# prs-eth/ResDepth

Measured on AMD Instinct MI355X. Metric: DSM tiles/sec fwd+bwd (256x256, 3-ch, depth-5 U-Net), higher is better.
Workload: dtype f32

## Files before the change

### resdepth_amd/csrc/rd_igemm.hip

```cpp
#include <stdlib.h>
#include <string.h>

#include <type_traits>

#include "rd_common.h"
#include "rd_mfma_dev.h"
#include "rd_nt.h"

namespace rd {

template <int BM, int BN, int WM, int WN, int AMODE, int EPI>
__global__ __launch_bounds__(256) void igemm_nt_kernel(NtParams p) {
    constexpr int BK = 32, LS = BK + 4;
    constexpr int TM = BM / WM / 32, TN = BN / WN / 32;
    constexpr int AI = BM / 32, BI = BN / 32;
    __shared__ __attribute__((aligned(16))) float smem[(BM + BN) * LS];
    float* As = smem;
    float* Bs = smem + BM * LS;

    const int lb = xcd_remap(blockIdx.x, gridDim.x);
    const int tile_n = lb % p.tiles_n, tile_m = lb / p.tiles_n;
    const int m0 = tile_m * BM, n0 = tile_n * BN;
    const int t = threadIdx.x, lane = t & 63, wave = t >> 6;
    const int wm = wave / WN, wn = wave % WN;
// ... 1090 lines not shown
        __syncthreads();
        for (long kb = k_begin; kb < k_end; kb += BK) {
            const bool more = kb + BK < k_end;
            if (more) load_tile(kb + BK);
#pragma unroll
            for (int ks = 0; ks < BK / 2; ++ks) {
                float af[TM], bf[TN];
#pragma unroll
                for (int i = 0; i < TM; ++i) af[i] = a_base[ks * 2 * BM + i * 32];
#pragma unroll
                for (int j = 0; j < TN; ++j) bf[j] = b_base[ks * 2 * BN + j * 32];
#pragma unroll
                for (int i = 0; i < TM; ++i)
#pragma unroll
                    for (int j = 0; j < TN; ++j)
                        acc[i][j] = __builtin_amdgcn_mfma_f32_32x32x2f32(af[i], bf[j], acc[i][j], 0, 0, 0);
            }
            __syncthreads();
            if (more) {
                store_tile();
                __syncthreads();
            }
        }
    }

    float* out = p.slab + (long)split * p.M * p.N;
#pragma unroll
    for (int i = 0; i < TM; ++i)
#pragma unroll
        for (int j = 0; j < TN; ++j) {
            const int n = n0 + wn * TN * 32 + j * 32 + lrow;
            if (n >= p.N) continue;
#pragma unroll
            for (int r = 0; r < 16; ++r) {
                const int m = m0 + wm * TM * 32 + i * 32 + (r & 3) + 8 * (r >> 2) + 4 * half;
                if (m < p.M) out[(long)m * p.N + n] = acc[i][j][r];
            }
        }
}

template <int NP, int BM, int BN, int WM, int WN, int AMODE, int BMODE>
__device__ __forceinline__ void wgrad_tn_split_body(const TnParams& p, float* smem, const Quant qz) {
    typedef typename frag_of<NP>::type FR;
    constexpr int NT = NP == 3 ? 2 : 3;
    constexpr int TM = BM / WM / 32, TN = BN / WN / 32;
    constexpr int STAGE = (BM + BN) * 32;

    const int nb_mn = p.tiles_mn;
    const int gb = xcd_remap(blockIdx.x, gridDim.x);
    const int split = gb / nb_mn;
    const int lb = gb - split * nb_mn;
    const int tile_n = lb % p.tiles_n, tile_m = lb / p.tiles_n;
    const int m0 = tile_m * BM, n0 = tile_n * BN;
    const int t = threadIdx.x, lane = t & 63, wave = t >> 6;
    const int wm = wave / WN, wn = wave % WN;
    const int H = p.H, W = p.W;

    const bool isA = t < BM, active = t < BM + BN;
    const int idx = isA ? t : t - BM;
    const int kq = idx & 3, quad = idx >> 2;
    const int col0 = (isA ? m0 : n0) + quad * 4;
    const bool col_ok = active && col0 < (isA ? p.M : p.N);
    int a_col = col0, a_qa = 0, a_qb = 0;
    if (AMODE == WA_UP2 && isA) {
        const int ab = col0 / p.Cout;
        a_col = col0 - ab * p.Cout;
        a_qa = ab >> 1;
        a_qb = ab & 1;
    }
    int b_col = col0, b_dy = 0, b_dx = 0;
    if (BMODE == WB_CONV3 && !isA) {
        const int tap = col0 / p.Cin;
        b_col = col0 - tap * p.Cin;
        b_dy = tap / 3 - 1;
        b_dx = tap - (tap / 3) * 3 - 1;
    }
    const int b_shift = b_dy * W + b_dx;
    const int lds_row0 = (isA ? 0 : BM) + quad * 4;

    f32x16 acc[TM][TN], lo[TM][TN];
#pragma unroll
    for (int i = 0; i < TM; ++i)
#pragma unroll
        for (int j = 0; j < TN; ++j)
#pragma unroll
            for (int r = 0; r < 16; ++r) acc[i][j][r] = lo[i][j][r] = 0.f;

    const long k_begin = (long)split * p.kchunk;
    long k_end = k_begin + p.kchunk;
    if (k_end > p.Kp) k_end = p.Kp;
    const __amdgpu_buffer_rsrc_t rsA = make_rsrc(p.A, p.a_bytes), rsB = make_rsrc(p.B, p.b_bytes);

    const bool w4 = (W & 3) == 0;
    auto load_task = [&](long kbase, float4 (&x)[4]) {
        const int rem = (int)(k_end - kbase);
        int img0 = 0, y0 = 0, x0 = 0;
        if ((AMODE == WA_UP2 && isA) || (BMODE == WB_CONV3 && !isA)) pix_split((int)kbase + kq * 4, p.pd, img0, y0, x0);
        unsigned up_off0 = 0;
        const unsigned up_step = (unsigned)(2 * p.lda * 4);
        if (AMODE == WA_UP2 && isA && w4)
            up_off0 = (unsigned)(((((long)img0 * (2 * H) + 2 * y0 + a_qa) * (2 * W) + 2 * x0 + a_qb) * p.lda + a_col) * 4);
#pragma unroll
        for (int j = 0; j < 4; ++j) {
            const int row = kq * 4 + j;
            const bool ok = col_ok && row < rem;
            if (isA) {
                if (AMODE == WA_UP2) {
                    unsigned off = up_off0 + j * up_step;
                    if (!w4) {
                        int jj, ii, img;
                        pix_split((int)kbase + row, p.pd, img, ii, jj);
                        off = (unsigned)(((((long)img * (2 * H) + 2 * ii + a_qa) * (2 * W) + 2 * jj + a_qb) * p.lda + a_col) * 4);
                    }
                    x[j] = buf_load4(rsA, ok ? off : kOOB, 0);
                } else {
                    x[j] = buf_load4(rsA, ok ? (unsigned)((row * p.lda + a_col) * 4) : kOOB, (unsigned)(kbase * p.lda * 4));
                }
            } else {
                if (BMODE == WB_CONV3) {
                    const int m = (int)kbase + row;
                    int y = y0, xx = x0 + j, img_ = img0;
                    if (!w4) pix_split(m, p.pd, img_, y, xx);
                    const bool in = ok && ((unsigned)(y + b_dy) < (unsigned)H) && ((unsigned)(xx + b_dx) < (unsigned)W);
                    x[j] = buf_load4(rsB, in ? (unsigned)((((long)m + b_shift) * p.ldb + b_col) * 4) : kOOB, 0);
                } else {
                    x[j] = buf_load4(rsB, ok ? (unsigned)((row * p.ldb + b_col) * 4) : kOOB, (unsigned)(kbase * p.ldb * 4));
                }
            }
        }
    };
    const float qs = __uint_as_float((unsigned)__builtin_amdgcn_readfirstlane((int)__float_as_uint(isA ? qz.sa : qz.sb)));
    auto store_task = [&](float* stage, const float4 (&x)[4]) {
        if (!active) return;
#pragma unroll
        for (int c = 0; c < 4; ++c) {
            uint2 ph, pm, pl;
            split_pack4v<NP, false>(c == 0 ? x[0].x : c == 1 ? x[0].y : c == 2 ? x[0].z : x[0].w, c == 0 ? x[1].x : c == 1 ? x[1].y : c == 2 ? x[1].z : x[1].w,
                                c == 0 ? x[2].x : c == 1 ? x[2].y : c == 2 ? x[2].z : x[2].w, c == 0 ? x[3].x : c == 1 ? x[3].y : c == 2 ? x[3].z : x[3].w,
                                qs, ph, pm, pl);
            const int row = lds_row0 + c;
            const int sw = (row >> 1) & 7;
            float* base = stage + row * 32 + (kq & 1) * 2;
            const int hi = kq >> 1;
            *reinterpret_cast<uint2*>(base + ((0 + hi) ^ sw) * 4) = ph;
            *reinterpret_cast<uint2*>(base + ((2 + hi) ^ sw) * 4) = pm;
            if (kterm3<NP>()) *reinterpret_cast<uint2*>(base + ((4 + hi) ^ sw) * 4) = pl;
        }
    };

    const int lrow = lane & 31, half = lane >> 5;
    int a_rd[TM][3], b_rd[TN][3];
#pragma unroll
    for (int i = 0; i < TM; ++i) {
        const int row = (wm * TM + i) * 32 + lrow;
#pragma unroll
        for (int q = 0; q < 3; ++q) a_rd[i][q] = row * 32 + ((2 * q + half) ^ ((row >> 1) & 7)) * 4;
    }
#pragma unroll
    for (int j = 0; j < TN; ++j) {
        const int row = BM + (wn * TN + j) * 32 + lrow;
#pragma unroll
        for (int q = 0; q < 3; ++q) b_rd[j][q] = row * 32 + ((2 * q + half) ^ ((row >> 1) & 7)) * 4;
    }
    auto mma_tile = [&](const float* stage) {
        FR af[TM][3], bf[TN][3];
#pragma unroll
        for (int i = 0; i < TM; ++i)
#pragma unroll
            for (int q = 0; q < NT; ++q) af[i][q] = *reinterpret_cast<const FR*>(stage + a_rd[i][q]);
#pragma unroll
        for (int j = 0; j < TN; ++j)
#pragma unroll
            for (int q = 0; q < NT; ++q) bf[j][q] = *reinterpret_cast<const FR*>(stage + b_rd[j][q]);
#pragma unroll
        for (int t6 = lo0<NP>(); t6 < 5; ++t6)
#pragma unroll
            for (int i = 0; i < TM; ++i)
#pragma unroll
                for (int j = 0; j < TN; ++j) lo[i][j] = mfma16<NP>(af[i][PA6[t6]], bf[j][PB6[t6]], lo[i][j]);
#pragma unroll
        for (int i = 0; i < TM; ++i)
#pragma unroll
            for (int j = 0; j < TN; ++j) acc[i][j] = mfma16<NP>(af[i][0], bf[j][0], acc[i][j]);
    };

    if (k_begin < k_end) {
        float* st0 = smem;
        float* st1 = smem + STAGE;
        float4 x0[4], x1[4];
        load_task(k_begin, x0);
        load_task(k_begin + SK, x1);
        store_task(st0, x0);
        __syncthreads();
        for (long kb = k_begin; kb < k_end; kb += 2 * SK) {
            load_task(kb + 2 * SK, x0);
            mma_tile(st0);
            store_task(st1, x1);
            __syncthreads();
            load_task(kb + 3 * SK, x1);
            mma_tile(st1);
            store_task(st0, x0);
            __syncthreads();
        }
    }

    float* out = p.slab + (long)split * p.M * p.N;
#pragma unroll
    for (int i = 0; i < TM; ++i)
#pragma unroll
        for (int j = 0; j < TN; ++j) {
            const int n = n0 + wn * TN * 32 + j * 32 + lrow;
            if (n >= p.N) continue;
#pragma unroll
            for (int r = 0; r < 16; ++r) {
                const int m = m0 + wm * TM * 32 + i * 32 + (r & 3) + 8 * (r >> 2) + 4 * half;
                if (m < p.M) out[(long)m * p.N + n] = merge_q<NP>(acc[i][j][r], lo[i][j][r], qz.dexp);
            }
        }
}

template <int BM, int BN, int WM, int WN, int AMODE, int BMODE>
__global__ __launch_bounds__(256) void wgrad_tn_split_kernel(TnParams p) {
    __shared__ __attribute__((aligned(16))) float smem[2 * (BM + BN) * 32];
    const Quant qz = quant_select(p.a_amax, p.b_amax);
    if (qz.use3) wgrad_tn_split_body<3, BM, BN, WM, WN, AMODE, BMODE>(p, smem, qz);
    else wgrad_tn_split_body<6, BM, BN, WM, WN, AMODE, BMODE>(p, smem, qz);
}

struct TnPlan {
    int bm, bn, tiles_m, tiles_n, splits, kchunk;
};

static TnPlan plan_tn(int M, int N, long Kp) {
    TnPlan pl;
    pl.bm = M > 64 ? 128 : 64;
    pl.bn = N > 64 ? 128 : 64;
    const int tforce = tune(TUNE_TN_TILE);
    if (tforce > 0) {
        pl.bm = tforce / 1000;
        pl.bn = tforce % 1000;
    }
    pl.tiles_m = cdiv(M, pl.bm);
    pl.tiles_n = cdiv(N, pl.bn);
    const int tiles = pl.tiles_m * pl.tiles_n;
    long ktiles = (Kp + 31) / 32;
    const int target = tune(TUNE_TN_BLOCKS);
    long want = target / tiles;
    if (want < 1) want = 1;
    long maxs = ktiles / 8 > 0 ? ktiles / 8 : 1;
    long s = want < maxs ? want : maxs;
    if (s < 1) s = 1;
    if (s > 512) s = 512;
    long per = (ktiles + s - 1) / s;
    pl.kchunk = (int)(per * 32);
    pl.splits = (int)((ktiles + per - 1) / per);
    return pl;
}

template <int AMODE, int BMODE>
static int launch_tn(TnParams p, const TnPlan& pl, hipStream_t s, const char* cls) {
    char pcls[64];
    const int tn_force = tune(TUNE_TN_SPLIT);
    const int split = tn_force >= 0 ? tn_force : (mfma_split() && pl.bm == 128 && pl.bn == 128);
    snprintf(pcls, sizeof(pcls), "%s|wgrad_tn%s<%d,%d,%d,%d>", cls, split ? "_split" : "", pl.bm, pl.bn, AMODE, BMODE);
    ProfScope ps(s, pcls, 2.0 * p.M * p.N * (double)p.Kp,
                 4.0 * ((double)p.Kp * p.lda * (AMODE == WA_UP2 ? 4 : 1) + (double)p.Kp * p.ldb + (double)p.M * p.N), true);
    const double a_bytes = 4.0 * (double)p.Kp * p.lda * (AMODE == WA_UP2 ? 4 : 1), b_bytes = 4.0 * (double)p.Kp * p.ldb;
    if (a_bytes >= 4294967040.0 || b_bytes >= 4294967040.0) {
        set_error("%s: operand larger than the 4 GiB buffer-descriptor range", cls);
        return RD_ERR_ARG;
    }
    p.a_bytes = (unsigned)a_bytes;
    p.b_bytes = (unsigned)b_bytes;
    p.kchunk = pl.kchunk;
    p.tiles_n = pl.tiles_n;
    p.tiles_mn = pl.tiles_m * pl.tiles_n;
    if (!split || mfma_products() != 3 || !p.a_amax || !p.b_amax) p.a_amax = p.b_amax = nullptr;
    const int grid = p.tiles_mn * pl.splits;
    if (split) {
        if (pl.bm == 128 && pl.bn == 128)
            RD_LAUNCH((wgrad_tn_split_kernel<128, 128, 2, 2, AMODE, BMODE>), dim3(grid), dim3(256), 0, s, p);
        else if (pl.bm == 128)
            RD_LAUNCH((wgrad_tn_split_kernel<128, 64, 2, 2, AMODE, BMODE>), dim3(grid), dim3(256), 0, s, p);
        else if (pl.bn == 128)
            RD_LAUNCH((wgrad_tn_split_kernel<64, 128, 2, 2, AMODE, BMODE>), dim3(grid), dim3(256), 0, s, p);
        else
            RD_LAUNCH((wgrad_tn_split_kernel<64, 64, 2, 2, AMODE, BMODE>), dim3(grid), dim3(256), 0, s, p);
        RD_LAUNCH_CHECK(cls);
        return RD_OK;
    }
    if (pl.bm == 128 && pl.bn == 128)
        RD_LAUNCH((wgrad_tn_kernel<128, 128, 2, 2, AMODE, BMODE>), dim3(grid), dim3(256), 0, s, p);
    else if (pl.bm == 128)
        RD_LAUNCH((wgrad_tn_kernel<128, 64, 2, 2, AMODE, BMODE>), dim3(grid), dim3(256), 0, s, p);
    else if (pl.bn == 128)
        RD_LAUNCH((wgrad_tn_kernel<64, 128, 2, 2, AMODE, BMODE>), dim3(grid), dim3(256), 0, s, p);
    else
        RD_LAUNCH((wgrad_tn_kernel<64, 64, 2, 2, AMODE, BMODE>), dim3(grid), dim3(256), 0, s, p);
    RD_LAUNCH_CHECK(cls);
    return RD_OK;
}

template <int SPT>
__global__ __launch_bounds__(256) void slab_reduce_kernel(const float* __restrict__ slab, float* __restrict__ dw, int M,
                                                          int N, int splits, int mode, int Cin, int Cout) {
    const long total = (long)M * N, quads = total >> 2;
    const long nthreads = (long)gridDim.x * blockDim.x;
    for (long gid = (long)blockIdx.x * blockDim.x + threadIdx.x; gid < quads * SPT; gid += nthreads) {
        const long q = gid / SPT;
        const int part = (int)(gid - q * SPT);
        const float4* src = reinterpret_cast<const float4*>(slab) + q;
        double a0 = 0.0, a1 = 0.0, a2 = 0.0, a3 = 0.0;
        int s = part;
        for (; s + 3 * SPT < splits; s += 4 * SPT) {
            const float4 v0 = src[(long)s * quads], v1 = src[(long)(s + SPT) * quads];
            const float4 v2 = src[(long)(s + 2 * SPT) * quads], v3 = src[(long)(s + 3 * SPT) * quads];
            a0 += ((double)v0.x + (double)v1.x) + ((double)v2.x + (double)v3.x);
            a1 += ((double)v0.y + (double)v1.y) + ((double)v2.y + (double)v3.y);
            a2 += ((double)v0.z + (double)v1.z) + ((double)v2.z + (double)v3.z);
            a3 += ((double)v0.w + (double)v1.w) + ((double)v2.w + (double)v3.w);
        }
        for (; s < splits; s += SPT) {
            const float4 v = src[(long)s * quads];
            a0 += v.x; a1 += v.y; a2 += v.z; a3 += v.w;
        }
#pragma unroll
        for (int o = 1; o < SPT; o <<= 1) {
            a0 += __shfl_xor(a0, o);
            a1 += __shfl_xor(a1, o);
            a2 += __shfl_xor(a2, o);
            a3 += __shfl_xor(a3, o);
        }
        if (part != 0) continue;
        const long e = q << 2;
        const int m = (int)(e / N), n = (int)(e - (long)m * N);
        const float r[4] = {(float)a0, (float)a1, (float)a2, (float)a3};
        if (mode == 3) {
            const int tq = n / Cout, co = n - tq * Cout;
#pragma unroll
            for (int k = 0; k < 4; ++k) dw[((long)(co + k) * Cin + m) * 9 + (8 - tq)] = r[k];
        } else if (mode == 2) {
            *reinterpret_cast<float4*>(dw + e) = make_float4(r[0], r[1], r[2], r[3]);
        } else if (mode == 0) {
            const int tap = n / Cin, ci = n - tap * Cin;
#pragma unroll
            for (int k = 0; k < 4; ++k) dw[((long)m * Cin + ci + k) * 9 + tap] = r[k];
        } else {
            const int ab = m / Cout, co = m - ab * Cout;
#pragma unroll
            for (int k = 0; k < 4; ++k) dw[((long)(n + k) * Cout + co) * 4 + ab] = r[k];
        }
    }
}

static void launch_slab_reduce(const float* slab, float* dw, int M, int N, int splits, int mode, int Cin, int Cout, hipStream_t s) {
#if RD_DIAG_SLAB_READ_DIV
    splits = (splits + RD_DIAG_SLAB_READ_DIV - 1) / RD_DIAG_SLAB_READ_DIV;
#endif
    const long quads = (long)M * N / 4;
    int spt = 1;
    while (spt < 16 && quads * spt < 262144 && 2 * spt <= splits) spt *= 2;
    const int grid = grid_for(quads * spt, 256, 4096);
    if (spt == 1) RD_LAUNCH(slab_reduce_kernel<1>, dim3(grid), dim3(256), 0, s, slab, dw, M, N, splits, mode, Cin, Cout);
    else if (spt == 2) RD_LAUNCH(slab_reduce_kernel<2>, dim3(grid), dim3(256), 0, s, slab, dw, M, N, splits, mode, Cin, Cout);
    else if (spt == 4) RD_LAUNCH(slab_reduce_kernel<4>, dim3(grid), dim3(256), 0, s, slab, dw, M, N, splits, mode, Cin, Cout);
    else if (spt == 8) RD_LAUNCH(slab_reduce_kernel<8>, dim3(grid), dim3(256), 0, s, slab, dw, M, N, splits, mode, Cin, Cout);
    else RD_LAUNCH(slab_reduce_kernel<16>, dim3(grid), dim3(256), 0, s, slab, dw, M, N, splits, mode, Cin, Cout);
}

__global__ void pack_conv3x3_kernel(const float* __restrict__ w, float* __restrict__ wf, float* __restrict__ wd,
                                    int cout, int cin) {
    const long total = (long)cout * cin * 9;
    for (long e = (long)blockIdx.x * blockDim.x + threadIdx.x; e < total; e += (long)gridDim.x * blockDim.x) {
        const int ci = (int)(e % cin);
        const int tap = (int)((e / cin) % 9);
        const int co = (int)(e / ((long)cin * 9));
        wf[e] = w[((long)co * cin + ci) * 9 + tap];
        if (wd) {
            const int co2 = (int)(e % cout);
            const int tap2 = (int)((e / cout) % 9);
            const int ci2 = (int)(e / ((long)cout * 9));
            wd[e] = w[((long)co2 * cin + ci2) * 9 + (8 - tap2)];
        }
    }
}

__global__ __launch_bounds__(256) void tiled_transpose_kernel(const float* __restrict__ in, float* __restrict__ out, int rows,
                                                              int groups, int cols, int flip) {
    __shared__ float tile[32][33];
    const int tiles_c = (cols + 31) / 32, tiles_r = (rows + 31) / 32;
    const int tx = threadIdx.x & 31, ty = threadIdx.x >> 5;
    for (long b = blockIdx.x; b < (long)groups * tiles_r * tiles_c; b += gridDim.x) {
        const int tc = (int)(b % tiles_c), tr = (int)((b / tiles_c) % tiles_r), g = (int)(b / ((long)tiles_c * tiles_r));
        const int r0 = tr * 32, c0 = tc * 32;
#pragma unroll
        for (int k = 0; k < 4; ++k) {
            const int r = r0 + ty + 8 * k, c = c0 + tx;
            tile[ty + 8 * k][tx] = (r < rows && c < cols) ? in[((long)r * groups + g) * cols + c] : 0.f;
        }
        __syncthreads();
        const int go = flip ? groups - 1 - g : g;
#pragma unroll
        for (int k = 0; k < 4; ++k) {
            const int c = c0 + ty + 8 * k, r = r0 + tx;
            if (r < rows && c < cols) out[((long)c * groups + go) * rows + r] = tile[tx][ty + 8 * k];
        }
        __syncthreads();
    }
}


__global__ void pack_convt_kernel(const float* __restrict__ w, float* __restrict__ wtf, float* __restrict__ wtd,
                                  int cin, int cout) {
    const long total = (long)cin * cout * 4;
    for (long e = (long)blockIdx.x * blockDim.x + threadIdx.x; e < total; e += (long)gridDim.x * blockDim.x) {
        const int ci = (int)(e % cin);
        const int co = (int)((e / cin) % cout);
        const int ab = (int)(e / ((long)cin * cout));
        wtf[e] = w[((long)ci * cout + co) * 4 + ab];
        if (wtd) {
            const int co2 = (int)(e % cout);
            const int ab2 = (int)((e / cout) % 4);
            const int ci2 = (int)(e / ((long)cout * 4));
            wtd[e] = w[((long)ci2 * cout + co2) * 4 + ab2];
        }
    }
}

static int grid_for(long total, int block = 256, int cap = 4096) {
    long g = (total + block - 1) / block;
    if (g > cap) g = cap;
    if (g < 1) g = 1;
    return (int)g;
}

static int check_conv_args(int n, int h, int w, int cin, int cout) {
    RD_REQUIRE(n > 0 && h > 0 && w > 0 && cin > 0 && cout > 0, "bad conv shape n=%d h=%d w=%d cin=%d cout=%d", n, h, w,
               cin, cout);
    RD_REQUIRE((long)n * h * w * 4L < (1L << 31), "pixel count too large for 32-bit tile indices");
    return RD_OK;
}

}

using namespace rd;

extern "C" {

int rd_mfma_products(void) { return mfma_products(); }

int rd_amax(const float* x, long long n, unsigned* slot, rd_stream_t s) {
    RD_REQUIRE(x && slot && n > 0, "rd_amax: bad arguments");
    launch_amax(x, (long)n, slot, nullptr, 1, (hipStream_t)s);
    RD_LAUNCH_CHECK("rd_amax");
    return RD_OK;
}


size_t rd_packed_weight_bytes(int rows, int taps, int cin) {
    if (rows <= 0 || taps <= 0 || cin <= 0) return 0;
    return packed_bytes(rows, taps, cin);
}

int rd_pack_conv3x3_weight(const float* w, float* wf, float* wd, int cout, int cin, rd_stream_t s) {
    RD_REQUIRE(w && wf && cout > 0 && cin > 0, "rd_pack_conv3x3_weight: bad arguments");
    ProfScope ps((hipStream_t)s, "pack_weights", 0, 12.0 * cout * cin * 9);
    unsigned* amax = mfma_products() == 3 ? quant_take().out2 : (quant_take(), nullptr);
    if (amax) launch_amax(w, (long)cout * cin * 9, amax, nullptr, 1, (hipStream_t)s);
    if (mfma_split()) {
        uint4* of = (uint4*)((char*)wf + packed_f32_bytes(cout, 9, cin));
        uint4* od = wd ? (uint4*)((char*)wd + packed_f32_bytes(cin, 9, cout)) : nullptr;
        const long pieces = rows32_of(cout) * nk16_of(9, cin) * 2 + (wd ? rows32_of(cin) * nk16_of(9, cout) * 2 : 0);
        long g = (pieces + 255) / 256;
        if (g > 8192) g = 8192;
        RD_LAUNCH(split_pack_conv3x3_kernel, dim3((int)g), dim3(256), 0, (hipStream_t)s, w, of, od, cout, cin,
                           (const float*)nullptr, (const unsigned*)amax);
        RD_LAUNCH_CHECK("pack_conv3x3");
        return RD_OK;
    }
    RD_LAUNCH(pack_conv3x3_kernel, dim3(grid_for((long)cout * cin * 9)), dim3(256), 0, (hipStream_t)s, w, wf,
                       (float*)nullptr, cout, cin);
    if (wd) {
        const long tiles = 9L * cdiv(cout, 32) * cdiv(cin, 32);
        RD_LAUNCH(tiled_transpose_kernel, dim3((int)(tiles < 8192 ? tiles : 8192)), dim3(256), 0, (hipStream_t)s,
                           (const float*)wf, wd, cout, 9, cin, 1);
    }
    RD_LAUNCH_CHECK("pack_conv3x3");
    if (int e = split_pack(wf, cout, 9, cin, (hipStream_t)s, amax)) return e;
    if (wd) return split_pack(wd, cin, 9, cout, (hipStream_t)s, amax);
    return RD_OK;
}

int rd_pack_conv3x3_weight_folded(const float* w, const float* row_scale, float* wf, int cout, int cin, rd_stream_t s) {
    RD_REQUIRE(w && wf && row_scale && cout > 0 && cin > 0, "rd_pack_conv3x3_weight_folded: bad arguments");
    RD_REQUIRE(mfma_split(), "rd_pack_conv3x3_weight_folded: only the split-bf16 kernels implement the folded inference path");
    ProfScope ps((hipStream_t)s, "pack_weights", 0, 10.0 * cout * cin * 9);
    unsigned* amax = mfma_products() == 3 ? quant_take().out2 : (quant_take(), nullptr);
    if (amax) launch_amax(w, (long)cout * cin * 9, amax, row_scale, (long)cin * 9, (hipStream_t)s);
    uint4* of = (uint4*)((char*)wf + packed_f32_bytes(cout, 9, cin));
    const long pieces = rows32_of(cout) * nk16_of(9, cin) * 2;
    long g = (pieces + 255) / 256;
    if (g > 8192) g = 8192;
    RD_LAUNCH(split_pack_conv3x3_kernel, dim3((int)g), dim3(256), 0, (hipStream_t)s, w, of, (uint4*)nullptr, cout, cin,
                       row_scale, (const unsigned*)amax);
    RD_LAUNCH_CHECK("pack_conv3x3_folded");
    return RD_OK;
}

long long rd_pack_item_pieces(int kind, int cout, int cin, int with_f32) {
    if (cout <= 0 || cin <= 0) return 0;
    if (kind == 0) return rows32_of(cout) * nk16_of(9, cin) * 2 + rows32_of(cin) * nk16_of(9, cout) * 2;
    return rows32_of(4L * cout) * nk16_of(1, cin) * 2 + rows32_of(cin) * nk16_of(4, cout) * 2 + (with_f32 ? (4L * cout * cin + 7) / 8 : 0);
}

long long rd_pack_item_tiles(int kind, int cout, int cin) {
    if (cout <= 0 || cin <= 0 || cout % 32 != 0 || cin % 32 != 0 || (kind != 0 && kind != 1)) return 0;
    return (long long)(cout / 32) * (cin / 32);
}

int rd_pack_weights_fused(const void* items_dev, int n_items, long long total_pieces, long long total_tiles, rd_stream_t s) {
    RD_REQUIRE(items_dev && n_items > 0 && total_pieces >= 0 && total_tiles >= 0 && total_pieces + total_tiles > 0,
               "rd_pack_weights_fused: bad arguments");
    RD_REQUIRE(mfma_split(), "rd_pack_weights_fused: the fused packer writes the split-bf16 operands only");
    ProfScope ps((hipStream_t)s, "pack_weights", 0, 10.0 * 8.0 * (double)total_pieces + 14.0 * 9216.0 * (double)total_tiles);
    if (mfma_products() == 3)
        RD_LAUNCH(pack_items_amax_kernel, dim3(AMAX_PARTS * n_items), dim3(256), 0, (hipStream_t)s, (const PackItem*)items_dev, n_items);
    if (total_tiles > 0) {
        const long gt = total_tiles < 4096 ? total_tiles : 4096;
        RD_LAUNCH(pack_tiles_kernel, dim3((int)gt), dim3(256), 0, (hipStream_t)s, (const PackItem*)items_dev, n_items,
                           (long)total_tiles);
    }
    if (total_pieces > 0) {
        long g = (total_pieces + 255) / 256;
        if (g > 16384) g = 16384;
        RD_LAUNCH(pack_all_kernel, dim3((int)g), dim3(256), 0, (hipStream_t)s, (const PackItem*)items_dev, n_items,
                           (long)total_pieces);
    }
    RD_LAUNCH_CHECK("pack_weights_fused");
    return RD_OK;
}

int rd_pack_convt2x2_weight(const float* w, float* wtf, float* wtd, int cin, int cout, rd_stream_t s) {
    RD_REQUIRE(w && wtf && cout > 0 && cin > 0, "rd_pack_convt2x2_weight: bad arguments");
    ProfScope ps((hipStream_t)s, "pack_weights", 0, 12.0 * cout * cin * 4);
    unsigned* amax = mfma_products() == 3 ? quant_take().out2 : (quant_take(), nullptr);
    if (amax) launch_amax(w, (long)cout * cin * 4, amax, nullptr, 1, (hipStream_t)s);
    RD_LAUNCH(pack_convt_kernel, dim3(grid_for((long)cout * cin * 4)), dim3(256), 0, (hipStream_t)s, w, wtf,
                       (float*)nullptr, cin, cout);
    if (wtd) {
        const long tiles = (long)cdiv(4 * cout, 32) * cdiv(cin, 32);
        RD_LAUNCH(tiled_transpose_kernel, dim3((int)(tiles < 8192 ? tiles : 8192)), dim3(256), 0, (hipStream_t)s,
                           (const float*)wtf, wtd, 4 * cout, 1, cin, 0);
    }
    RD_LAUNCH_CHECK("pack_convt");
    if (int e = split_pack(wtf, 4L * cout, 1, cin, (hipStream_t)s, amax)) return e;
    if (wtd) return split_pack(wtd, cin, 4, cout, (hipStream_t)s, amax);
    return RD_OK;
}

int rd_conv3x3_fwd(const float* x, const float* wf, float* z, int n, int h, int w, int cin, int cout, rd_stream_t s) {
    return rd_conv3x3_fwd_stats(x, wf, z, nullptr, n, h, w, cin, cout, nullptr, 0, s);
}

size_t rd_conv3x3_fwd_stats_ws_bytes(int n, int h, int w, int cin, int cout) {
    (void)cin;
    return (size_t)cdiv((long)n * h * w, 64) * 2 * cout * sizeof(float);
}

int rd_conv3x3_fwd_stats(const float* x, const float* wf, float* z, double* sums, int n, int h, int w, int cin, int cout,
                         void* ws, size_t ws_bytes, rd_stream_t s) {
    if (int e = check_conv_args(n, h, w, cin, cout)) return e;
    RD_REQUIRE(x && wf && z, "rd_conv3x3_fwd: null pointer");
    RD_REQUIRE(cin % 4 == 0, "rd_conv3x3_fwd: Cin must be a multiple of 4 (got %d); use rd_conv3x3_first_fwd", cin);
    if (sums && (!ws || ws_bytes < rd_conv3x3_fwd_stats_ws_bytes(n, h, w, cin, cout))) {
        set_error("rd_conv3x3_fwd_stats: workspace too small");
        return RD_ERR_WS;
    }
    NtParams p = {};
    set_quant(p, quant_take());
    p.A = x; p.B = wf; p.C = z;
    p.M = n * h * w; p.N = cout; p.K = 9 * cin; p.Cin = cin;
    p.H = h; p.W = w; p.pd = make_pixdiv(h, w);
    p.stats = sums ? (float*)ws : nullptr;
    int tiles_m = 0;
    if (int e = launch_nt<A_CONV3, EPI_STORE>(p, (hipStream_t)s, "conv3x3_fwd", &tiles_m)) return e;
    if (sums) return reduce_partials_f32((const float*)ws, sums, tiles_m, 2 * cout, (hipStream_t)s);
    return RD_OK;
}

int rd_conv3x3_fwd_bn(const float* x, const float* wf, float* z, double count, float eps, float momentum, float* mean,
                      float* invstd, float* running_mean, float* running_var, int64_t* nbt, int n, int h, int w, int cin,
                      int cout, void* ws, size_t ws_bytes, rd_stream_t s) {
    if (int e = check_conv_args(n, h, w, cin, cout)) return e;
    RD_REQUIRE(x && wf && z && mean && invstd && count > 0, "rd_conv3x3_fwd_bn: bad arguments");
    RD_REQUIRE(cin % 4 == 0, "rd_conv3x3_fwd_bn: Cin must be a multiple of 4 (got %d); use rd_conv3x3_first_fwd_bn", cin);
    if (!ws || ws_bytes < rd_conv3x3_fwd_stats_ws_bytes(n, h, w, cin, cout)) {
        set_error("rd_conv3x3_fwd_bn: workspace too small");
        return RD_ERR_WS;
    }
    NtParams p = {};
    set_quant(p, quant_take());
    p.A = x; p.B = wf; p.C = z;
    p.M = n * h * w; p.N = cout; p.K = 9 * cin; p.Cin = cin;
    p.H = h; p.W = w; p.pd = make_pixdiv(h, w);
    p.stats = (float*)ws;
    int tiles_m = 0;
    if (int e = launch_nt<A_CONV3, EPI_STORE>(p, (hipStream_t)s, "conv3x3_fwd", &tiles_m)) return e;
    return bn_reduce_finalize((const float*)ws, tiles_m, cout, count, eps, momentum, mean, invstd, running_mean, running_var, nbt,
                              (hipStream_t)s);
}

int rd_conv3x3_fwd_act(const float* x, const float* wf_folded, const float* shift, float slope, float* a, float* pooled, int n,
                       int h, int w, int cin, int cout, rd_stream_t s) {
    if (int e = check_conv_args(n, h, w, cin, cout)) return e;
    RD_REQUIRE(x && wf_folded && shift && a, "rd_conv3x3_fwd_act: null pointer");
    RD_REQUIRE(cin % 4 == 0 && cout % 4 == 0, "rd_conv3x3_fwd_act: channels must be multiples of 4 (%d, %d)", cin, cout);
    RD_REQUIRE(mfma_split(), "rd_conv3x3_fwd_act: only the split-bf16 kernels implement the folded inference path");
    RD_REQUIRE(!pooled || (w % 16 == 0 && h % 8 == 0),
               "rd_conv3x3_fwd_act: the pooling epilogue needs W a multiple of 16 and H a multiple of 8 (got %dx%d)", h, w);
    NtParams p = {};
    set_quant(p, quant_take_img());
    p.A = x; p.B = wf_folded; p.C = a;
    p.M = n * h * w; p.N = cout; p.K = 9 * cin; p.Cin = cin;
    p.H = h; p.W = w; p.pd = make_pixdiv(h, w);
    p.shift = shift; p.act_slope = slope; p.pool_out = pooled;
    return launch_nt<A_CONV3, EPI_STORE>(p, (hipStream_t)s, "conv3x3_fwd");
}

int rd_conv3x3_bwd_data(const float* dz, const float* wd, float* dx, int n, int h, int w, int cin, int cout,
                        rd_stream_t s) {
    if (int e = check_conv_args(n, h, w, cin, cout)) return e;
    RD_REQUIRE(dz && wd && dx, "rd_conv3x3_bwd_data: null pointer");
    RD_REQUIRE(cout % 4 == 0, "rd_conv3x3_bwd_data: Cout must be a multiple of 4 (got %d)", cout);
    NtParams p = {};
    set_quant(p, quant_take());
    p.A = dz; p.B = wd; p.C = dx;
    p.M = n * h * w; p.N = cin; p.K = 9 * cout; p.Cin = cout;
    p.H = h; p.W = w; p.pd = make_pixdiv(h, w);
    return launch_nt<A_CONV3, EPI_STORE>(p, (hipStream_t)s, "conv3x3_dgrad");
}

static int set_bn_hook(NtParams& p, const char* who, const float* bn_z, const float* mean, const float* invstd, const float* gamma,
                       const float* beta, float slope, const float* slope_dev, int mode, float* part, size_t part_floats) {
    RD_REQUIRE(bn_z && mean && invstd && gamma && beta && part && (mode == 1 || mode == 2), "%s: bad BN-statistics arguments", who);
    RD_REQUIRE(p.N % 4 == 0, "%s: the BN-statistics epilogue needs a multiple of 4 channels (got %d)", who, p.N);
    RD_REQUIRE(part_floats >= rd_bn_bwd_part_floats(p.M, p.N), "%s: statistics buffer too small (%zu < %zu floats)", who,
               part_floats, rd_bn_bwd_part_floats(p.M, p.N));
    p.bn_z = bn_z; p.bn_mean = mean; p.bn_invstd = invstd; p.bn_gamma = gamma; p.bn_beta = beta;
    p.bn_slope = slope; p.bn_slope_dev = slope_dev; p.bn_mode = mode; p.bn_part = part;
    return RD_OK;
}

size_t rd_bn_bwd_part_floats(long long pixels, int c) { return (size_t)cdiv(pixels, 64) * 4 * (size_t)c; }

int rd_conv3x3_bwd_data_bnstats(const float* dz, const float* wd, float* dx, int n, int h, int w, int cin, int cout,
                                const float* bn_z, const float* mean, const float* invstd, const float* gamma,
                                const float* beta, float slope, const float* slope_dev, int mode, float* part,
                                size_t part_floats, int* rows_out, rd_stream_t s) {
    if (int e = check_conv_args(n, h, w, cin, cout)) return e;
    RD_REQUIRE(dz && wd && dx && rows_out, "rd_conv3x3_bwd_data_bnstats: null pointer");
    RD_REQUIRE(cout % 4 == 0, "rd_conv3x3_bwd_data_bnstats: Cout must be a multiple of 4 (got %d)", cout);
    NtParams p = {};
    set_quant(p, quant_take());
    p.A = dz; p.B = wd; p.C = dx;
    p.M = n * h * w; p.N = cin; p.K = 9 * cout; p.Cin = cout;
    p.H = h; p.W = w; p.pd = make_pixdiv(h, w);
    if (int e = set_bn_hook(p, "rd_conv3x3_bwd_data_bnstats", bn_z, mean, invstd, gamma, beta, slope, slope_dev, mode, part,
                            part_floats))
        return e;
    return launch_nt<A_CONV3, EPI_STORE>(p, (hipStream_t)s, "conv3x3_dgrad", rows_out);
// ... 255 lines not shown
```

Before: 4551.

## Stage split-K weight-gradient reduction through LDS tiles for coalesced scattered stores

Adds a tiled slab-reduce kernel for the three scattered output layouts (modes 0, 1 and 3). Each block reduces the split-K partial sums for a tile, writes them into shared memory, and then writes contiguous runs of the final weight gradient, using float4 when the destination is aligned. This replaces the strided 9- or 4-element scatter writes of the old kernel. The cost is shared-memory staging, a barrier, and block sizes of 576 threads, which may lower parallelism for small layers.

```diff
diff --git a/resdepth_amd/csrc/rd_igemm.hip b/resdepth_amd/csrc/rd_igemm.hip
--- a/resdepth_amd/csrc/rd_igemm.hip
+++ b/resdepth_amd/csrc/rd_igemm.hip
@@ -1416,6 +1416,32 @@
 }
 
 template <int SPT>
+__device__ __forceinline__ void slab_sum_quad(const float4* __restrict__ src, long stride, int splits, int part, bool live,
+                                              double (&a)[4]) {
+    a[0] = a[1] = a[2] = a[3] = 0.0;
+    if (live) {
+        int s = part;
+        for (; s + 3 * SPT < splits; s += 4 * SPT) {
+            const float4 v0 = src[(long)s * stride], v1 = src[(long)(s + SPT) * stride];
+            const float4 v2 = src[(long)(s + 2 * SPT) * stride], v3 = src[(long)(s + 3 * SPT) * stride];
+            a[0] += ((double)v0.x + (double)v1.x) + ((double)v2.x + (double)v3.x);
+            a[1] += ((double)v0.y + (double)v1.y) + ((double)v2.y + (double)v3.y);
+            a[2] += ((double)v0.z + (double)v1.z) + ((double)v2.z + (double)v3.z);
+            a[3] += ((double)v0.w + (double)v1.w) + ((double)v2.w + (double)v3.w);
+        }
+        for (; s < splits; s += SPT) {
+            const float4 v = src[(long)s * stride];
+            a[0] += v.x; a[1] += v.y; a[2] += v.z; a[3] += v.w;
+        }
+    }
+#pragma unroll
+    for (int o = 1; o < SPT; o <<= 1) {
+#pragma unroll
+        for (int k = 0; k < 4; ++k) a[k] += __shfl_xor(a[k], o);
+    }
+}
+
+template <int SPT>
 __global__ __launch_bounds__(256) void slab_reduce_kernel(const float* __restrict__ slab, float* __restrict__ dw, int M,
                                                           int N, int splits, int mode, int Cin, int Cout) {
     const long total = (long)M * N, quads = total >> 2;
@@ -1423,32 +1449,12 @@
     for (long gid = (long)blockIdx.x * blockDim.x + threadIdx.x; gid < quads * SPT; gid += nthreads) {
         const long q = gid / SPT;
         const int part = (int)(gid - q * SPT);
-        const float4* src = reinterpret_cast<const float4*>(slab) + q;
-        double a0 = 0.0, a1 = 0.0, a2 = 0.0, a3 = 0.0;
-        int s = part;
-        for (; s + 3 * SPT < splits; s += 4 * SPT) {
-            const float4 v0 = src[(long)s * quads], v1 = src[(long)(s + SPT) * quads];
-            const float4 v2 = src[(long)(s + 2 * SPT) * quads], v3 = src[(long)(s + 3 * SPT) * quads];
-            a0 += ((double)v0.x + (double)v1.x) + ((double)v2.x + (double)v3.x);
-            a1 += ((double)v0.y + (double)v1.y) + ((double)v2.y + (double)v3.y);
-            a2 += ((double)v0.z + (double)v1.z) + ((double)v2.z + (double)v3.z);
-            a3 += ((double)v0.w + (double)v1.w) + ((double)v2.w + (double)v3.w);
-        }
-        for (; s < splits; s += SPT) {
-            const float4 v = src[(long)s * quads];
-            a0 += v.x; a1 += v.y; a2 += v.z; a3 += v.w;
-        }
-#pragma unroll
-        for (int o = 1; o < SPT; o <<= 1) {
-            a0 += __shfl_xor(a0, o);
-            a1 += __shfl_xor(a1, o);
-            a2 += __shfl_xor(a2, o);
-            a3 += __shfl_xor(a3, o);
-        }
+        double a[4];
+        slab_sum_quad<SPT>(reinterpret_cast<const float4*>(slab) + q, quads, splits, part, true, a);
         if (part != 0) continue;
         const long e = q << 2;
         const int m = (int)(e / N), n = (int)(e - (long)m * N);
-        const float r[4] = {(float)a0, (float)a1, (float)a2, (float)a3};
+        const float r[4] = {(float)a[0], (float)a[1], (float)a[2], (float)a[3]};
         if (mode == 3) {
             const int tq = n / Cout, co = n - tq * Cout;
 #pragma unroll
@@ -1465,6 +1471,104 @@
             for (int k = 0; k < 4; ++k) dw[((long)(n + k) * Cout + co) * 4 + ab] = r[k];
         }
     }
+}
+
+template <int SPT>
+struct SlabTile {
+    static constexpr int QW = 64 / SPT;
+    static constexpr int CQ = 8, ROWS = QW / CQ;
+    static constexpr bool FLAT_OK = QW >= 8, TR_OK = ROWS >= 4;
+};
+
+template <int SPT, int P, bool TR>
+__global__ __launch_bounds__(64 * P) void slab_reduce_tile_kernel(const float* __restrict__ slab, float* __restrict__ dw,
+                                                                  long quads, int splits, int R, int C, long row_stride,
+                                                                  long plane_stride, int flip, int tiles_c, int vec) {
+    using T = SlabTile<SPT>;
+    constexpr int RUN = (TR ? T::ROWS : 4 * T::QW) * P, PITCH = TR ? RUN + 4 : RUN, NRUN = TR ? 4 * T::CQ : 1;
+    __shared__ __align__(16) float tile[NRUN * PITCH];
+    const int plane = threadIdx.x >> 6, lane = threadIdx.x & 63;
+    const int ql = lane / SPT, part = lane - ql * SPT;
+    const int pt = flip ? P - 1 - plane : plane;
+    const int tr = TR ? blockIdx.x / tiles_c : 0;
+    const int r0 = tr * T::ROWS, c0 = TR ? (blockIdx.x - tr * tiles_c) * T::CQ * 4 : 0;
+    const long f0 = TR ? 0 : (long)blockIdx.x * T::QW * 4;
+    int row, col, l0;
+    bool live;
+    if (TR) {
+        const int r = ql / T::CQ, cq = ql - r * T::CQ;
+        row = r0 + r;
+        col = c0 + cq * 4;
+        live = row < R && col < C;
+        l0 = 4 * cq * PITCH + r * P + pt;
+    } else {
+        const long f = f0 + ql * 4;
+        live = f < (long)R * C;
+        row = (int)(f / C);
+        col = (int)(f - (long)row * C);
+        l0 = 4 * ql * P + pt;
+    }
+    const long off = live ? row * row_stride + plane * plane_stride + col : 0;
+    double a[4];
+    slab_sum_quad<SPT>(reinterpret_cast<const float4*>(slab + off), quads, splits, part, live, a);
+    if (live && part == 0) {
+#pragma unroll
+        for (int k = 0; k < 4; ++k) tile[l0 + k * (TR ? PITCH : P)] = (float)a[k];
+    }
+    __syncthreads();
+    int runs, len;
+    if (TR) {
+        runs = C - c0 < NRUN ? C - c0 : NRUN;
+        len = (R - r0 < T::ROWS ? R - r0 : T::ROWS) * P;
+    } else {
+        const long left = (long)R * C - f0;
+        runs = 1;
+        len = (int)(left < 4 * T::QW ? left : 4 * T::QW) * P;
+    }
+    if (vec) {
+        for (int i = threadIdx.x; i < NRUN * (RUN / 4); i += 64 * P) {
+            const int c = i / (RUN / 4), t = (i - c * (RUN / 4)) * 4;
+            if (c < runs && t < len) {
+                float* dst = dw + (TR ? ((long)(c0 + c) * R + r0) * P : f0 * P) + t;
+                *reinterpret_cast<float4*>(dst) = *reinterpret_cast<const float4*>(tile + c * PITCH + t);
+            }
+        }
+    } else {
+        for (int i = threadIdx.x; i < NRUN * RUN; i += 64 * P) {
+            const int c = i / RUN, t = i - c * RUN;
+            if (c < runs && t < len) dw[(TR ? ((long)(c0 + c) * R + r0) * P : f0 * P) + t] = tile[c * PITCH + t];
+        }
+    }
+}
+
+template <int SPT>
+static void launch_slab_reduce_spt(const float* slab, float* dw, int M, int N, int splits, int mode, int Cin, int Cout, hipStream_t s) {
+    using T = SlabTile<SPT>;
+    const long quads = (long)M * N / 4;
+    const int vec = (reinterpret_cast<uintptr_t>(dw) & 15) == 0;
+    if constexpr (T::FLAT_OK) {
+        if (mode == 0) {
+            RD_LAUNCH((slab_reduce_tile_kernel<SPT, 9, false>), dim3(cdiv((long)Cout * Cin / 4, T::QW)), dim3(576), 0, s, slab, dw,
+                      quads, splits, Cout, Cin, 9L * Cin, (long)Cin, 0, 1, vec);
+            return;
+        }
+    }
+    if constexpr (T::TR_OK) {
+        if (mode == 3) {
+            const int tiles_c = cdiv(Cout / 4, T::CQ);
+            RD_LAUNCH((slab_reduce_tile_kernel<SPT, 9, true>), dim3(tiles_c * cdiv(Cin, T::ROWS)), dim3(576), 0, s, slab, dw,
+                      quads, splits, Cin, Cout, 9L * Cout, (long)Cout, 1, tiles_c, vec);
+            return;
+        }
+        if (mode == 1) {
+            const int tiles_c = cdiv(Cin / 4, T::CQ);
+            RD_LAUNCH((slab_reduce_tile_kernel<SPT, 4, true>), dim3(tiles_c * cdiv(Cout, T::ROWS)), dim3(256), 0, s, slab, dw,
+                      quads, splits, Cout, Cin, (long)Cin, (long)Cout * Cin, 0, tiles_c, vec);
+            return;
+        }
+    }
+    RD_LAUNCH(slab_reduce_kernel<SPT>, dim3(grid_for(quads * SPT, 256, 4096)), dim3(256), 0, s, slab, dw, M, N, splits, mode, Cin,
+              Cout);
 }
 
 static void launch_slab_reduce(const float* slab, float* dw, int M, int N, int splits, int mode, int Cin, int Cout, hipStream_t s) {
@@ -1474,12 +1578,11 @@
     const long quads = (long)M * N / 4;
     int spt = 1;
     while (spt < 16 && quads * spt < 262144 && 2 * spt <= splits) spt *= 2;
-    const int grid = grid_for(quads * spt, 256, 4096);
-    if (spt == 1) RD_LAUNCH(slab_reduce_kernel<1>, dim3(grid), dim3(256), 0, s, slab, dw, M, N, splits, mode, Cin, Cout);
-    else if (spt == 2) RD_LAUNCH(slab_reduce_kernel<2>, dim3(grid), dim3(256), 0, s, slab, dw, M, N, splits, mode, Cin, Cout);
-    else if (spt == 4) RD_LAUNCH(slab_reduce_kernel<4>, dim3(grid), dim3(256), 0, s, slab, dw, M, N, splits, mode, Cin, Cout);
-    else if (spt == 8) RD_LAUNCH(slab_reduce_kernel<8>, dim3(grid), dim3(256), 0, s, slab, dw, M, N, splits, mode, Cin, Cout);
-    else RD_LAUNCH(slab_reduce_kernel<16>, dim3(grid), dim3(256), 0, s, slab, dw, M, N, splits, mode, Cin, Cout);
+    if (spt == 1) launch_slab_reduce_spt<1>(slab, dw, M, N, splits, mode, Cin, Cout, s);
+    else if (spt == 2) launch_slab_reduce_spt<2>(slab, dw, M, N, splits, mode, Cin, Cout, s);
+    else if (spt == 4) launch_slab_reduce_spt<4>(slab, dw, M, N, splits, mode, Cin, Cout, s);
+    else if (spt == 8) launch_slab_reduce_spt<8>(slab, dw, M, N, splits, mode, Cin, Cout, s);
+    else launch_slab_reduce_spt<16>(slab, dw, M, N, splits, mode, Cin, Cout, s);
 }
 
 __global__ void pack_conv3x3_kernel(const float* __restrict__ w, float* __restrict__ wf, float* __restrict__ wd,
```

New measurement: 4579, median of 6. No clear change (+0.6%).
